# nghiapq77/face-recognition-cpp-tensorrt

Measured on AMD Instinct MI355X. Metric: faces/sec end-to-end (detect+embed+match), 640x640 batch=32, 1M gallery, higher is better.
Workload: dtype f16 MFMA recogniser convs (fp32 accumulate) + fp32-accurate detector (fp32 MFMA, fp16 hi/lo-split MFMA for the 64-channel 3x3 convs) + int8-screened coarse scan (fp16 MFMA on exactly widened int8 rows) + exact f32 re-rank match (bit-identical to the exact f32 scan)

## Files before the change

### face-recognition-cpp-tensorrt_amd/csrc/frt_kernels.h

```cpp
#pragma once
#include <hip/hip_runtime.h>
#include <stdint.h>

#include <vector>

#include "../../include/frt.h"
#include "frt_faces.hpp"

typedef _Float16 half_t;
typedef _Float16 half8 __attribute__((ext_vector_type(8)));
typedef _Float16 half4 __attribute__((ext_vector_type(4)));
typedef float floatx16 __attribute__((ext_vector_type(16)));
typedef float floatx4 __attribute__((ext_vector_type(4)));

constexpr int FRT_MAX_DEVICES = 32;
inline bool frt_first_use_on_device(bool (&done)[FRT_MAX_DEVICES]) {
    int d = 0;
    (void)hipGetDevice(&d);
    d &= FRT_MAX_DEVICES - 1;
    if (done[d]) return false;
    done[d] = true;
    return true;
}

void launch_spin(double microseconds, hipStream_t s);
double launch_mfma_probe(int mix, int n_wg, int iters, const void *src, float *out, hipStream_t s);

struct MatchPartial {
    float sim;
    int32_t idx;
};
template <typename GT>
void launch_match_top1(const GT *rows, int N, int D, const float *queries, int F, MatchPartial *partial, int partial_blocks, int32_t *idx_out,
                       float *sim_out, int row_offset, hipStream_t s);
int match_top1_blocks(int N, int F);
template <typename GT>
void launch_match_full(const GT *rows, int N, int D, const float *queries, int F, float *out, hipStream_t s);
constexpr int FRT_MATCH_COARSE_WG = 256;
constexpr int FRT_MATCH_SEL_SUB = 64;
constexpr int FRT_MATCH_CTL_WORDS = 32 + FRT_MATCH_SEL_SUB * 32;
struct MatchPair {
    int q, tile;
};
constexpr int FRT_MATCH_PAIR_TILE_MASK = (1 << 28) - 1;
constexpr int FRT_MATCH_CTL_OVERFLOW = 1, FRT_MATCH_CTL_SEG0 = 32, FRT_MATCH_CTL_STRIDE = 32;
struct ScreenScratch {
    float *tilemax;
    float *wgmax;
    void *pairs;
    int pair_cap;
    int *ctl;
    unsigned long long *qkey;
    const uint8_t *g8;
    const float *g8_scale;
    float gerr;
};
size_t gallery8_bytes(int N, int D);
void launch_gallery_shadow8(const float *gallery, int N, int D, uint8_t *g8, float *scale, int *max_err2_bits, int *max_norm2_bits, hipStream_t s);
void launch_gallery_shadow(const float *gallery, int N, int D, half_t *g16, int *max_norm2_bits, hipStream_t s);
void launch_match_screened(const float *gallery, const half_t *g16, int N, int D, const float *queries, int F, int k, float gmax_norm,
                           const ScreenScratch &w, float *kth_scratch, MatchPartial *partial, int partial_blocks, int32_t *idx_out, float *sim_out,
                           int row_offset, hipStream_t s);
void launch_match_topk(const float *gallery, const half_t *g16, int N, int D, const float *queries, int F, int k, bool screen, float gmax_norm,
                       const ScreenScratch &w, float *kth_scratch, MatchPartial *partial, int partial_blocks, int32_t *idx_out, float *sim_out,
                       int row_offset, hipStream_t s);
int match_topk_max();
bool launch_match_coarse(const half_t *g16, int N, int D, const float *queries, int F, const ScreenScratch &w, hipStream_t s);
void launch_match_select_threshold(int N, int D, const float *queries, int F, float threshold, int tile_min, float gmax_norm, const ScreenScratch &w, bool i8,
                                   hipStream_t s);
void launch_match_topk_labels(const float *gallery, const half_t *g16, int N, int D, const float *queries, int F, int k, int kth_count, float gmax_norm,
                              const ScreenScratch &w, float *kth_scratch, MatchPartial *partial, int partial_blocks, const int32_t *labels,
                              int32_t *label_out, int32_t *idx_out, float *sim_out, int row_offset, hipStream_t s);
void launch_half_to_float(const half_t *in, long n, float *out, hipStream_t s);
void launch_float_to_half(const float *in, long n, half_t *out, hipStream_t s);
void launch_merge_topk(const int32_t *idx_all, const float *sim_all, int shards, int n, int k, int32_t *idx_out, float *sim_out, hipStream_t s);
void launch_merge_topk_labels(const int32_t *label_all, const int32_t *idx_all, const float *sim_all, int shards, int n, int k, int32_t *label_out,
                              int32_t *idx_out, float *sim_out, hipStream_t s);
size_t gallery16_elems(int N, int D);
__device__ __forceinline__ long g16_index(long g, int k, int D) {
    return ((((g >> 7) * 4 + ((g >> 5) & 3)) * (long)(D >> 4) + (k >> 4)) * 64 + ((k >> 3) & 1) * 32 + (g & 31)) * 8 + (k & 7);
}
__device__ __forceinline__ floatx4 load_g4(const float *G, long g, int D, int k) { return *reinterpret_cast<const floatx4 *>(G + g * D + k); }
__device__ __forceinline__ floatx4 load_g4(const half_t *G, long g, int D, int k) {
    const half4 h = *reinterpret_cast<const half4 *>(G + g16_index(g, k, D));
    return floatx4{(float)h[0], (float)h[1], (float)h[2], (float)h[3]};
}
template <typename GT>
__device__ __forceinline__ float exact_row_dot(const GT *__restrict__ G, long g, int D, const float *q) {
    float acc = 0.f;
#pragma unroll 8
    for (int k0 = 0; k0 < D; k0 += 8) {
        const floatx4 a = load_g4(G, g, D, k0), b = load_g4(G, g, D, k0 + 4);
        const floatx4 x = *reinterpret_cast<const floatx4 *>(q + k0), y = *reinterpret_cast<const floatx4 *>(q + k0 + 4);
#pragma unroll
        for (int s2 = 0; s2 < 4; ++s2) {
            acc = __builtin_fmaf(a[s2], x[s2], acc);
            acc = __builtin_fmaf(b[s2], y[s2], acc);
        }
    }
    return acc;
}
bool match_screen_supported(int D);
void launch_rows_to_half(const float *in, long row0, long n_rows, int D, half_t *g16, hipStream_t s);
template <typename GT>
void launch_rows_norm(const GT *G, int row0, int n_rows, int D, int *max_norm2_bits, hipStream_t s);
void launch_gallery_shadow8_rows(const float *rows, int row0, int n_rows, uint8_t *g8, float *scale, int *max_err2_bits, int *max_norm2_bits, hipStream_t s);
void launch_gather_rows(const float *G, int D, int a, int n_rows, const int *keys, int klo, int khi, float *bounce, hipStream_t s);
void launch_gather_rows16(const half_t *G, int D, long tile0, long n_tiles, int n_new, const int *keys, int klo, int khi, half_t *bounce, hipStream_t s);

void launch_cluster_init(int32_t *parent, int N, long long *stats, hipStream_t s);
void launch_cluster_queries(const half_t *rows, int row0, int n, int D, float *out, hipStream_t s);
template <typename GT>
void launch_cluster_rerank_union(const GT *rows, int N, int D, const float *queries, int q_row0, int tile_origin, const ScreenScratch &w, float t,
                                 int32_t *parent, long long *stats, int *chunk_overflow, hipStream_t s);
void launch_cluster_dense_union(const float *full, int F, int N, int q_row0, float t, int32_t *parent, long long *stats, hipStream_t s);
void launch_cluster_flatten(const int32_t *parent, int N, int32_t *labels, long long *stats, long long screened_chunks, long long dense_chunks,
                            hipStream_t s);

constexpr int FRT_SEPARATION_MAX_THRESHOLDS = 64;
void launch_match_select_kth(int N, int D, const float *queries, int F, int kth_count, float gmax_norm, const ScreenScratch &w, float *kth_scratch, bool i8,
                             hipStream_t s);
void launch_match_top1_excluding(const float *gallery, const half_t *g16, int N, int D, const float *queries, int F, bool screened, const ScreenScratch &w,
                                 MatchPartial *partial, int partial_blocks, const int32_t *labels, const int32_t *excluded, int32_t *idx_out, float *sim_out,
                                 int *overflow_out, hipStream_t s);
template <typename GT>
void launch_separation_genuine(const GT *rows, int N, int D, const int *group_off, const int *group_rows, const int *pos_ident, float *gen_sim,
                               int32_t *gen_row, hipStream_t s);
void launch_separation_reduce(const float *gen_sim, const int32_t *gen_row, const float *imp_sim, const int32_t *imp_row, int N, const float *thresholds,
                              int n_thresholds, const int *chunk_overflow, int chunks, bool screened, long long *counts, long long *stats, hipStream_t s);

template <typename GT>
void launch_template_build(const GT *rows, int D, const int *group_off, const int *group_rows, int I, int row_offset, float *templates, float *min_sim,
                           int32_t *min_row, hipStream_t s);

constexpr int DET_MAX_LEVELS = 4, DET_MAX_SIZES = 3;
struct DetGeom {
    int in_w, in_h, frame_w, frame_h;
    int levels;
    int fw[DET_MAX_LEVELS], fh[DET_MAX_LEVELS];
    int base[DET_MAX_LEVELS];
    int nsz[DET_MAX_LEVELS];
    int min_size[DET_MAX_LEVELS][DET_MAX_SIZES];
    float step[DET_MAX_LEVELS];
    int A;
    float scale_w, scale_h;
    float nms_thr, bbox_thr;
    int max_faces;
};
DetGeom det_geometry(int family, int levels, int in_w, int in_h, int frame_w, int frame_h, float nms_threshold, float bbox_threshold, int max_faces);
struct Candidate {
    frt_bbox box;
    int32_t anchor;
};
void launch_decode(const float *loc, const float *conf, int n_frames, const DetGeom &g, Candidate *cand, int *cand_count, hipStream_t s);
void launch_nms(Candidate *cand, const float *loc, int *cand_count, int n_frames, const DetGeom &g, uint8_t *dead, frt_bbox *out, int *n_out,
                int *kept_anchor, hipStream_t s);
void launch_landmark_decode(const float *ldm, const int *kept_anchor, const int *n_out, int n_frames, const DetGeom &g, float *out, hipStream_t s);
void launch_align_faces(const uint8_t *frames, int frame_h, int frame_w, size_t row_stride, size_t frame_stride, const float *landmarks,
                        const int *n_boxes, int max_faces, int F, int frames_shared, uint8_t *crops, float *chw, int *valid, hipStream_t s);

void launch_det_preprocess(const uint8_t *frames, int n, int frame_h, int frame_w, size_t row_stride, size_t frame_stride, int in_h,
                           int in_w, float *out, hipStream_t s);
void launch_crop_faces(const uint8_t *frames, int frame_h, int frame_w, size_t row_stride, size_t frame_stride, const frt_bbox *boxes,
                       const int *n_boxes, int max_faces, int F, int frames_shared, int oh, int ow, uint8_t *crops, float *chw, int *valid,
                       hipStream_t s);
void launch_resize_linear(const uint8_t *src, int n, int sh, int sw, size_t sstride, size_t sframe, uint8_t *dst, int dh, int dw, size_t dstride,
                          size_t dframe, hipStream_t s);
void launch_face_normalize(const uint8_t *crops, int F, int oh, int ow, float *chw, hipStream_t s);
void launch_faces_prepare(const uint8_t *arena, const frt_face_desc *desc, int F, uint8_t *crops, float *chw, hipStream_t s);
void launch_images_resize(const uint8_t *arena, const frt_face_desc *desc, int n, int dh, int dw, uint8_t *out, hipStream_t s);

void launch_cut_tiles(const uint8_t *photo, int rows, int cols, size_t row_stride, const frt_tile *tiles, int n_tiles, int tile_rows, int tile_cols,
                      uint8_t *out, hipStream_t s);
struct TileMergeArgs {
    const frt_bbox *boxes;
    const int32_t *n_boxes;
    const frt_tile *tiles;
    int n_tiles, slots, photo_rows, photo_cols, tile_rows, tile_cols, metric, drop_cut;
    float thr;
    int max_out;
    unsigned long long *keys;
    frt_bbox *mbox;
    int *order;
    unsigned long long *mask;
    frt_bbox *out;
    int32_t *src_out;
    int *n_out;
};
size_t tile_merge_mask_words(int candidates);
void launch_tile_merge(const TileMergeArgs &a, hipStream_t s);
void launch_tile_landmarks(const float *ldm, const frt_tile *tiles, const int32_t *src, const int *n_out, int slots, int max_out, int photo_rows,
                           int photo_cols, int tile_rows, int tile_cols, float *out, hipStream_t s);
void launch_tile_faces_select(const frt_bbox *boxes, const int32_t *src, const float *ldm, const int *n_in, int cap, int min_face, int max_batch,
                              frt_bbox *boxes_kept, int32_t *src_kept, float *ldm_kept, int32_t *keep_pos, int *n_kept, int32_t *pass_count,
                              hipStream_t s);

void launch_enrol_select(const frt_face_result *results, const float *embeds, int n_frames, int max_faces, int32_t *status, frt_face_result *face_out,
                         float *rows, int32_t *count, hipStream_t s, const struct frt_face_quality *quality = nullptr);

void launch_face_quality(const uint8_t *crops, const frt_face_result *results, int n, const frt_quality_options &opt, struct frt_face_quality *out,
                         hipStream_t s);

struct DwPwArgs {
    const float *in; float *out;
    const float *wd, *bd;
    const float *wp, *bp;
    const float *add;
    int add_h, add_w;
    int B, Cin, H, W, Cout, Ho, Wo, stride, relu;
    float *tmp;
    const float *wd12;
    const half_t *wph;
    const float *wdp;
    const half_t *wpf;
    const float *wdt;
    const float *stem;
    const float *zeros;
};
size_t dwpw_wave_zero_bytes();
bool launch_dwpw_wave(const DwPwArgs &a, hipStream_t s);
void launch_dwpw(const DwPwArgs &a, hipStream_t s);
bool launch_dwpw_mfma(const DwPwArgs &a, hipStream_t s);
struct Conv3Args {
    const float *in; float *out;
    const float *w, *b;
    int B, Cin, H, W, Cout, Ho, Wo, stride, relu;
    int out_ctotal, out_coff;
    const half_t *wh;
    float *out2;
    int split, out2_ctotal, out2_coff;
};
void launch_conv3x3(const Conv3Args &a, hipStream_t s);
size_t det_stem_weight_floats();
void det_stem_pack(const Conv3Args &c, const DwPwArgs &d1, const DwPwArgs &d2, float *dst, hipStream_t s);
bool launch_det_stem(const uint8_t *frames, size_t row_stride, size_t frame_stride, const Conv3Args &c, const DwPwArgs &d1, const DwPwArgs &d2, hipStream_t s);
bool launch_det_conv1_u8(const uint8_t *frames, size_t row_stride, size_t frame_stride, const Conv3Args &a, hipStream_t s);
bool launch_conv3x3_split(const Conv3Args *a, int n, hipStream_t s);
void launch_conv3x3_multi(const Conv3Args *a, int n, hipStream_t s);
struct HeadArgs {
    const float *in;
    const float *wb, *bb;
    const float *wc, *bc;
    float *loc, *conf;
    int B, C, H, W, A, base;
    const float *wl, *bl;
    float *ldm;
};
void launch_heads(const HeadArgs &a, hipStream_t s);
void launch_heads_multi(const HeadArgs *a, int n, hipStream_t s);

struct SlimHeadArgs {
    const float *in;
    const float *wd;
    const float *wp, *bp;
    int C, H, W, na, base;
};
struct SlimHeadsArgs {
    SlimHeadArgs lv[3];
    float *loc, *conf, *ldm;
    int B, A;
};
void launch_slim_heads(const SlimHeadsArgs &a, int n, hipStream_t s);
struct DenseHeadArgs {
    const float *in;
    const float *w, *b;
    float *loc, *conf, *ldm;
    int B, C, H, W, na, cout, cpad, A, base;
};
void launch_dense_head(const DenseHeadArgs &a, hipStream_t s);
struct RfbProjArgs {
    const float *in;
    const float *w, *b;
    float *red, *sc;
    int B, H, W;
};
void launch_rfb_proj(const RfbProjArgs &a, hipStream_t s);
struct RfbConvArgs {
    const float *in; float *out;
    const float *w, *b;
    int Cin, Cout, dil, relu, in_ctotal, in_coff, out_ctotal, out_coff;
};
struct RfbConvMulti {
    RfbConvArgs p[3];
    int B, H, W;
};
void launch_rfb_conv(const RfbConvMulti &a, int n, hipStream_t s);
struct RfbTailArgs {
    const float *cat;
    const float *w, *b;
    const float *sc;
    float *out;
    float scale;
    int B, H, W;
};
void launch_rfb_tail(const RfbTailArgs &a, hipStream_t s);

enum { EPI_PRELU = 0, EPI_BN = 1, EPI_BN_ADD_BN = 2, EPI_PARTIAL = 3, EPI_BN_SE = 4 };
struct ConvMfmaArgs {
    const half_t *x;
    const half_t *w;
    const half_t *wf;
    const half_t *wf2;
    int B, H, W, Cin, Ho, Wo, Cout, ks, stride, pad;
    int mode;
    const float *p0, *p1, *p2, *p3;
    const half_t *sc;
    int sc_h, sc_w, sc_stride;
    const half_t *scx;
    const half_t *wscf;
    const float *psc0, *psc1;
    int Csc;
    half_t *out0, *out1;
    float *outf;
    int splits;
    const half_t *zeros;
    float *se_pool;
    const float *se_w1, *se_w2;
    int *se_counter;
    int se_flag_off;
    int se_epoch;
    int *se_error;
    const int *strip_tab;
    int strip_period, strip_ppx;
};
struct StripGeometry {
    int H, W;
    int compact;
    int linear;
    int nt;
    int R;
    int n_img;
    int nslot;
    int threads;
};
struct StripTables {
    int period = 0;
    int ppx = 0;
    int stride = 0;
    std::vector<int> data;
};
constexpr int strip_table_stride(const StripGeometry &g) { return g.nslot * g.threads + g.nt * 64 + (g.compact ? g.nt * 4 : g.nt * 32); }
StripTables strip_tables(const StripGeometry &g);
enum ConvFamily { CONV_SMALL, CONV_KS, CONV_C64, CONV_S2, CONV_STRIP };
struct ConvPlan {
    int family = CONV_STRIP;
    int row = 0;
    const char *label = "";
    int R = 0, n_img = 1;
    int M = 0;
    bool uses_scx = false;
    int se_row = -1;
    const char *se_label = nullptr;
    bool se_fused() const { return se_row >= 0; }
    void take_se_tail() { row = se_row; label = se_label; }
};
struct ConvRow {
    const char *label;
    void (*launch)(const ConvMfmaArgs &a, const ConvPlan &p, hipStream_t s);
    int se_row;
};
inline void conv_plan_row(ConvPlan &p, int family, const ConvRow *table, int row) {
    p.family = family;
    p.row = row;
    p.label = table[row].label;
}
inline void conv_plan_se_twin(ConvPlan &p, const ConvRow *table, const ConvMfmaArgs &a) {
    if (table[p.row].se_row < 0 || a.mode != EPI_BN_ADD_BN || !a.se_pool || !a.sc || !a.out1) return;
    p.se_row = table[p.row].se_row;
    p.se_label = table[p.se_row].label;
}
ConvPlan conv_plan(const ConvMfmaArgs &a);
bool conv_strip_geometry(const ConvMfmaArgs &a, const ConvPlan &p, StripGeometry &g);
void conv_strip_tables_warm(const ConvMfmaArgs &a, const ConvPlan &p);
void launch_conv_mfma(const ConvMfmaArgs &a, const ConvPlan &p, hipStream_t s);
bool conv_se_fits_device();
bool plan_small(const ConvMfmaArgs &a, ConvPlan &p);
void launch_small(const ConvMfmaArgs &a, const ConvPlan &p, hipStream_t s);
bool plan_ks(const ConvMfmaArgs &a, ConvPlan &p);
void launch_ks(const ConvMfmaArgs &a, const ConvPlan &p, hipStream_t s);
bool plan_c64(const ConvMfmaArgs &a, ConvPlan &p);
void launch_c64(const ConvMfmaArgs &a, const ConvPlan &p, hipStream_t s);
bool plan_s2(const ConvMfmaArgs &a, ConvPlan &p);
void launch_s2(const ConvMfmaArgs &a, const ConvPlan &p, hipStream_t s);
struct ArcInputArgs {
    const float *x;
    const float *w;
    const float *s0, *b0;
    const float *slope;
    const float *s1, *b1;
    half_t *y, *z;
    int F, H, W;
    const half_t *wh;
};
void launch_arc_input(const ArcInputArgs &a, hipStream_t s);
bool launch_arc_input_mfma(const ArcInputArgs &a, hipStream_t s);
void launch_fc_slices(const half_t *z, const half_t *wfrag, int F, float *partial, hipStream_t s);
struct Conv32Args {
    const float *x, *w, *ps, *pb;
    float *out;
    int F, H, W, Cin, Ho, Wo, Cout, ks, stride, pad, mode;
    const float *p0, *p1, *sc;
    int sc_h, sc_w, sc_stride;
};
void launch_arc32_input(const float *x, const float *w, const float *s0, const float *b0, const float *slope, float *y, int F, hipStream_t s);
void launch_conv32(const Conv32Args &c, hipStream_t s);
void pack_conv32_weights(const float *w, int cout, int taps, int cin, float *out);
void launch_fc32(const float *y, const float *sn, const float *bn, const float *w, float *out, int F, hipStream_t s);
void launch_se32(const float *res, const float *w1, const float *w2, float *gate, const float *sc, float *out, int F, int Ho, int Wo, int C, int sc_h, int sc_w, int sc_stride,
                 hipStream_t s);
void launch_fc_finalize(const float *partial, int splits, int F, const float *bias, const float *s, const float *b, const int *valid,
                        float *out, hipStream_t s_);
void launch_arc_flip_pair(const float *chw, float *pair, int n, hipStream_t s);
void launch_arc_flip_mirror(const float *chw, float *mirror, int n, hipStream_t s);
void launch_fc_finalize_pair(const float *partial_a, const float *partial_b, int splits, int rows, int n, const float *bias, const float *s, const float *b,
                             const int *valid, float *out, hipStream_t s_);
struct SeArgs {
    const half_t *res;
    const float *w1;
    const float *w2;
    const half_t *sc; int sc_h, sc_w, sc_stride;
    const float *s1, *b1;
    half_t *y, *z;
    float *pool;
    float *gate;
    int F, H, W, C;
    int *counter;
};
void launch_se(const SeArgs &a, hipStream_t s);

constexpr int FRT_TRACK_MAX_FRAMES = 256, FRT_TRACK_MAX_STREAMS = 1024, FRT_TRACK_MAX_SLOTS = 64, FRT_TRACK_MAX_DIM = 2048;
struct TrackStreamIds {
    uint16_t id[FRT_TRACK_MAX_FRAMES];
};
struct TrackArgs {
    frt_track_state *slots;
    float *sums;
    int32_t *counters;
    int max_tracks, max_faces, dim;
    float iou_threshold, decay;
    int max_missed, min_hits;
    const frt_face_result *results;
    const float *embeds;
    frt_track_result *tracks;
    float *templates;
    float reid_threshold, iou_min_sim;
    float *sim;
    unsigned long long *sim_defined;
    frt_track_assoc *assoc;
};
void launch_track_similarity(const TrackArgs &a, const TrackStreamIds &ids, int n_frames, hipStream_t s);
void launch_track_update(const TrackArgs &a, const TrackStreamIds &ids, int n_frames, bool appearance, hipStream_t s);
void launch_track_identity(const TrackArgs &a, const TrackStreamIds &ids, int n_frames, const int32_t *idx, const float *sim, hipStream_t s);
void launch_track_reset(const TrackArgs &a, int n_streams, int stream, hipStream_t s);
```

### face-recognition-cpp-tensorrt_amd/csrc/kernels_det_wave.hip

```cpp
#include <cstdlib>
#include <type_traits>
#include <utility>

#include "frt_kernels.h"

namespace {

typedef float floatx2 __attribute__((ext_vector_type(2)));
typedef _Float16 half2v __attribute__((ext_vector_type(2)));
typedef unsigned uint2v __attribute__((ext_vector_type(2)));
typedef unsigned uint4v __attribute__((ext_vector_type(4)));
typedef unsigned uint16v __attribute__((ext_vector_type(16)));

__device__ __forceinline__ int xcd_tile(int nblocks) {
    const int bq = nblocks >> 3, brem = nblocks & 7;
    const int xcd = blockIdx.x & 7, slot = blockIdx.x >> 3;
    return (xcd < brem ? xcd * (bq + 1) : brem * (bq + 1) + (xcd - brem) * bq) + slot;
}

template <int CIN, int NCB, int H, int W, int STRIDE, int NBUF_>
struct WaveGeom {
    static constexpr int WO = W / STRIDE, HO = H / STRIDE;
    static constexpr int HW = H * W, HOWO = HO * WO;
    static constexpr int SPAN = (WO + 62) / WO + 1;
    static constexpr int ROWS = STRIDE * (SPAN - 1) + 3;
    static constexpr int SL = W / 4 + 1;
    static constexpr int CPC = 8;
    static constexpr int SPC = CPC / 4;
    static constexpr int CHS = SL * 16;
    static constexpr int ROWB = CPC * CHS + (W % 32) * 4;
    static constexpr int CHUNKB = ROWS * ROWB;
    static constexpr int NDR = (CPC * SL + 63) / 64;
    static constexpr int DMAOPS = ROWS * NDR;
    static constexpr int NBUF = NBUF_, LA = NBUF_ - 1;
    static constexpr int NCHUNK = CIN / CPC, NG = CIN / 16, NSTEP = CIN / 4;
    static constexpr int NA = 2 * NCB;
    static constexpr int LDS_BYTES = NBUF * CHUNKB + 16;
    static_assert(SPC == 2 && CIN % 16 == 0 && CHS / 4 + 2 < 256 && LA >= 2, "shape not covered");
    static constexpr int younger(int cw) {
        const int at_step = cw == 0 ? -1 : 2 * cw - 2;
        int n = 0;
        bool seen = false;
        for (int k = 0; k < LA; ++k) {
            if (seen) n += DMAOPS;
            if (k == cw) seen = true;
        }
        if (seen) n += NA;
        for (int st = 0; st <= at_step; ++st) {
            if ((st & 1) == 0 && st / 2 + LA < NCHUNK) {
                if (seen) n += DMAOPS;
                if (st / 2 + LA == cw) seen = true;
            }
            if (st < at_step && (st & 3) == 3 && st / 4 + 1 < NG && seen) n += NA;
        }
        return n;
    }
};

template <int I, int N, class F>
__device__ __forceinline__ void static_for(F &&f) {
    if constexpr (I < N) {
        f(std::integral_constant<int, I>{});
        static_for<I + 1, N>(f);
    }
}

template <int N>
__device__ __forceinline__ void wait_vm() {
    static_assert(N >= 0 && N < 64, "vmcnt is a 6-bit counter");
#ifdef WAVE_VM0
    asm volatile("s_waitcnt vmcnt(0)" ::: "memory");
#else
    asm volatile("s_waitcnt vmcnt(%0)" ::"n"(N) : "memory");
#endif

}

struct WaveArgs {
    const float *in; float *out;
    const float *bp, *wdp;
    const half_t *wpf;
    const float *zeros;
#ifdef WAVE_STAMP
    long long *stamps;
#endif
};
#ifdef WAVE_STAMP
#define WSTAMP(i) do { if (blockIdx.x == 0 && threadIdx.x == 0) a.stamps[i] = __builtin_readcyclecounter(); } while (0)
#else
#define WSTAMP(i) do { } while (0)
#endif

template <int CIN, int COUT, int NCB, int H, int W, int STRIDE, int NBUF>
__global__ __launch_bounds__(64) __attribute__((amdgpu_num_sgpr(48))) void dwpw_wave_kernel(WaveArgs a) {
    using G = WaveGeom<CIN, NCB, H, W, STRIDE, NBUF>;
    extern __shared__ __attribute__((aligned(16))) char lds[];
    const int lane = threadIdx.x, r = lane & 31, hi = lane >> 5;
    constexpr int HW = G::HW, HoWo = G::HOWO;
    constexpr int tpi = (HoWo + 63) >> 6;
    const int lid = xcd_tile(gridDim.x);
    const int b = lid / tpi, p0 = (lid - b * tpi) * 64;
    const int y_first = p0 / G::WO;
    const int cob = (int)blockIdx.y * NCB;

    WSTAMP(0);
    for (int o = lane * 16; o < G::LDS_BYTES; o += 1024) *reinterpret_cast<floatx4 *>(lds + o) = floatx4{0.f, 0.f, 0.f, 0.f};
    asm volatile("s_waitcnt lgkmcnt(0)" ::: "memory");

    unsigned voff[G::NDR];
    bool lval[G::NDR];
#pragma unroll
    for (int i = 0; i < G::NDR; ++i) {
        const int q = lane + 64 * i, k = q / G::SL, sl = q - k * G::SL;
        lval[i] = q < G::CPC * G::SL && sl >= 1;
        voff[i] = lval[i] ? (unsigned)((k * HW + (sl - 1) * 4) * 4) : 0u;
    }
    const char *rsrc[G::ROWS];
    unsigned rstep[G::ROWS];
    {
        const char *inb = reinterpret_cast<const char *>(a.in + (long)b * CIN * HW);
        const char *zer = reinterpret_cast<const char *>(a.zeros);
#pragma unroll
        for (int j = 0; j < G::ROWS; ++j) {
            const int iy = y_first * STRIDE - 1 + j;
            const bool in = iy >= 0 && iy < H;
            rsrc[j] = in ? inb + iy * W * 4 : zer;
            rstep[j] = in ? (unsigned)(G::CPC * HW * 4) : 0u;
        }
    }
    const unsigned lds0 = (unsigned)(uintptr_t)(__attribute__((address_space(3))) char *)lds;
    auto dma_chunk = [&](auto cc) {
        constexpr int c = decltype(cc)::value;
#pragma unroll
        for (int i = 0; i < G::NDR; ++i)
            if (lval[i]) {
                const unsigned vo = voff[i];
#pragma unroll
                for (int j = 0; j < G::ROWS; ++j) {
                    const char *src = rsrc[j];
                    const unsigned dst = lds0 + (c % G::NBUF) * G::CHUNKB + j * G::ROWB + i * 1024;
                    asm volatile("s_mov_b32 m0, %2\n\tglobal_load_lds_dwordx4 %0, %1" ::"v"(vo), "s"(src), "s"(dst) : "memory");
                }
            }
#pragma unroll
        for (int j = 0; j < G::ROWS; ++j) rsrc[j] += rstep[j];
    };

    const int pl = min(p0 + lane, HoWo - 1);
    const int oy = pl / G::WO, ox = pl - oy * G::WO;
    const unsigned rb = (unsigned)(uintptr_t)(__attribute__((address_space(3))) char *)lds +
                        (unsigned)(((oy - y_first) * STRIDE) * G::ROWB + (ox * STRIDE + 3) * 4);

    half8 ah[2][NCB], al[2][NCB];
    const half_t *wf = a.wpf + (long)lane * 8;
    const int ncb_total = COUT / 32;
    auto load_a = [&](auto gc) {
        constexpr int g = decltype(gc)::value;
#pragma unroll
        for (int cb = 0; cb < NCB; ++cb) {
            const half_t *p = wf + ((long)(g * ncb_total + cob + cb) * 2) * 512;
            ah[g & 1][cb] = *reinterpret_cast<const half8 *>(p);
            al[g & 1][cb] = *reinterpret_cast<const half8 *>(p + 512);
        }
    };

    floatx16 acc[2][NCB];
#pragma unroll
    for (int t = 0; t < 2; ++t)
#pragma unroll
        for (int cb = 0; cb < NCB; ++cb)
#pragma unroll
            for (int e = 0; e < 16; ++e) acc[t][cb][e] = 0.f;

    floatx4 bias4[NCB][4];
    WSTAMP(1);
    asm volatile("" ::: "memory");
    static_for<0, G::LA>(dma_chunk);
    asm volatile("" ::: "memory");
    load_a(std::integral_constant<int, 0>{});
    asm volatile("" ::: "memory");

    floatx2 tv[2][2][9];
    auto issue_taps3 = [&](auto qc, auto dc, floatx2(&v)[9]) {
        constexpr int q = decltype(qc)::value, d = decltype(dc)::value;
        constexpr int c = q / (G::CPC / 2), pr = q % (G::CPC / 2);
        constexpr int boff = (c % G::NBUF) * G::CHUNKB + 2 * pr * G::CHS + d * G::ROWB;
        const unsigned b0 = rb + boff;
        asm volatile("ds_read2_b32 %0, %3 offset0:0 offset1:%4\n"
                     "ds_read2_b32 %1, %3 offset0:1 offset1:%5\n"
                     "ds_read2_b32 %2, %3 offset0:2 offset1:%6"
                     : "=&v"(v[3 * d]), "=&v"(v[3 * d + 1]), "=&v"(v[3 * d + 2])
                     : "v"(b0), "n"(G::CHS / 4), "n"(G::CHS / 4 + 1), "n"(G::CHS / 4 + 2)
                     : "memory");
    };
    auto issue_taps = [&](auto qc, floatx2(&v)[9]) {
        issue_taps3(qc, std::integral_constant<int, 0>{}, v);
        issue_taps3(qc, std::integral_constant<int, 1>{}, v);
        issue_taps3(qc, std::integral_constant<int, 2>{}, v);
    };
    auto landed = [&](floatx2(&u)[9], floatx2(&v)[9]) {
        asm volatile("s_waitcnt lgkmcnt(0)"
                     : "+v"(u[0]), "+v"(u[1]), "+v"(u[2]), "+v"(u[3]), "+v"(u[4]), "+v"(u[5]), "+v"(u[6]), "+v"(u[7]), "+v"(u[8])::"memory");
        asm volatile("" : "+v"(v[0]), "+v"(v[1]), "+v"(v[2]), "+v"(v[3]), "+v"(v[4]), "+v"(v[5]), "+v"(v[6]), "+v"(v[7]), "+v"(v[8])::"memory");
    };
#define WAVE_W_CLOBBERS                                                                                                                            \
    "s56", "s57", "s58", "s59", "s60", "s61", "s62", "s63", "s64", "s65", "s66", "s67", "s68", "s69", "s70", "s71", "s72", "s73", "s74", "s75", "s76", \
        "s77", "s78", "s79", "s80", "s81", "s82", "s83", "s84", "s85", "s86", "s87", "s88", "s89", "s90", "s91", "s92", "s93", "s94", "s95"
    const float *wdp = a.wdp;
    auto load_w = [&](auto sc) {
        constexpr int st = decltype(sc)::value;
        const float *wsrc = wdp;
        asm volatile("s_load_dwordx16 s[56:71], %0, %1\n"
                     "s_load_dwordx4 s[72:75], %0, %2\n"
                     "s_load_dwordx16 s[76:91], %0, %3\n"
                     "s_load_dwordx4 s[92:95], %0, %4" ::"s"(wsrc),
                     "n"(st * 160), "n"(st * 160 + 64), "n"(st * 160 + 80), "n"(st * 160 + 144)
                     : "memory", WAVE_W_CLOBBERS);
    };
    const floatx2 ones = {1.f, 1.f};
    auto chain3 = [&](auto jc, floatx2 &oa, floatx2 &ob, floatx2(&u)[9], floatx2(&v)[9]) {
        constexpr int j = decltype(jc)::value;
        const floatx2 one2 = ones;
        if constexpr (j == 0)
            asm volatile("v_pk_mul_f32 %0, %8, s[74:75]\n"
                         "v_pk_mul_f32 %1, %8, s[94:95]\n"
                         "v_pk_fma_f32 %0, %2, s[56:57], %0\n"
                         "v_pk_fma_f32 %1, %5, s[76:77], %1\n"
                         "v_pk_fma_f32 %0, %3, s[58:59], %0\n"
                         "v_pk_fma_f32 %1, %6, s[78:79], %1\n"
                         "v_pk_fma_f32 %0, %4, s[60:61], %0\n"
                         "v_pk_fma_f32 %1, %7, s[80:81], %1"
                         : "=&v"(oa), "=&v"(ob)
                         : "v"(u[0]), "v"(u[1]), "v"(u[2]), "v"(v[0]), "v"(v[1]), "v"(v[2]), "v"(one2)
                         : "memory");
        else if constexpr (j == 1)
            asm volatile("v_pk_fma_f32 %0, %2, s[62:63], %0\n"
                         "v_pk_fma_f32 %1, %5, s[82:83], %1\n"
                         "v_pk_fma_f32 %0, %3, s[64:65], %0\n"
                         "v_pk_fma_f32 %1, %6, s[84:85], %1\n"
                         "v_pk_fma_f32 %0, %4, s[66:67], %0\n"
                         "v_pk_fma_f32 %1, %7, s[86:87], %1"
                         : "+v"(oa), "+v"(ob)
                         : "v"(u[3]), "v"(u[4]), "v"(u[5]), "v"(v[3]), "v"(v[4]), "v"(v[5])
                         : "memory");
        else
            asm volatile("v_pk_fma_f32 %0, %2, s[68:69], %0\n"
                         "v_pk_fma_f32 %1, %5, s[88:89], %1\n"
                         "v_pk_fma_f32 %0, %3, s[70:71], %0\n"
                         "v_pk_fma_f32 %1, %6, s[90:91], %1\n"
                         "v_pk_fma_f32 %0, %4, s[72:73], %0\n"
                         "v_pk_fma_f32 %1, %7, s[92:93], %1"
                         : "+v"(oa), "+v"(ob)
                         : "v"(u[6]), "v"(u[7]), "v"(u[8]), "v"(v[6]), "v"(v[7]), "v"(v[8])
                         : "memory");
    };

    {
        const float *wsrc = wdp;
        static_for<0, (CIN * 10 * 4 + 63) / 64>([&](auto ic) {
            unsigned sink;
            const float *src2 = wsrc;
            asm volatile("s_load_dword %0, %1, %2" : "=s"(sink) : "s"(src2), "n"(decltype(ic)::value * 64) : "memory");
        });
        asm volatile("s_waitcnt lgkmcnt(0)" ::: "memory");
    }
    WSTAMP(2);
    wait_vm<G::younger(0)>();
    asm volatile("s_sleep 2" ::: "memory");
    WSTAMP(3);
    load_w(std::integral_constant<int, 0>{});
    issue_taps(std::integral_constant<int, 0>{}, tv[0][0]);
    issue_taps(std::integral_constant<int, 1>{}, tv[0][1]);

    unsigned hp[8], lp[8];
    half8 pbh[2], pbl[2];
    constexpr int MF_STEP = 3 * 2 * NCB / 4;
    auto mfma_n = [&](auto gc, auto mc) {
        constexpr int g = decltype(gc)::value, m = decltype(mc)::value;
        constexpr int round = m / (2 * NCB), t = (m / NCB) % 2, cb = m % NCB;
#ifndef WAVE_NO_MFMA
        acc[t][cb] = __builtin_amdgcn_mfma_f32_32x32x16_f16(round == 2 ? al[g & 1][cb] : ah[g & 1][cb], round == 1 ? pbl[t] : pbh[t], acc[t][cb], 0, 0, 0);
#else
        acc[t][cb][round] += (float)pbh[t][cb] + (float)pbl[t][cb] + (float)ah[g & 1][cb][round] + (float)al[g & 1][cb][round];
#endif
    };
    auto step = [&](auto sc) {
        constexpr int st = decltype(sc)::value;
        constexpr int c = st / 2, g = st / 4, k = st % 4;
        if constexpr ((st & 1) == 0 && c + G::LA < G::NCHUNK) dma_chunk(std::integral_constant<int, c + G::LA>{});
        if constexpr ((st & 1) == 0 && c + 1 < G::NCHUNK) wait_vm<G::younger(c + 1)>();
        if constexpr (st == G::NSTEP - 2) {
#pragma unroll
            for (int cb = 0; cb < NCB; ++cb)
#pragma unroll
                for (int kq = 0; kq < 4; ++kq) bias4[cb][kq] = *reinterpret_cast<const floatx4 *>(a.bp + (cob + cb) * 32 + 8 * kq + 4 * hi);
        }
        WSTAMP(7 + st);
        floatx2 oa, ob;
        landed(tv[st & 1][0], tv[st & 1][1]);
        chain3(std::integral_constant<int, 0>{}, oa, ob, tv[st & 1][0], tv[st & 1][1]);
        chain3(std::integral_constant<int, 1>{}, oa, ob, tv[st & 1][0], tv[st & 1][1]);
        chain3(std::integral_constant<int, 2>{}, oa, ob, tv[st & 1][0], tv[st & 1][1]);
        if constexpr (st + 1 < G::NSTEP) load_w(std::integral_constant<int, st + 1>{});
        static_for<0, 6>([&](auto ic) {
            constexpr int i = decltype(ic)::value;
            if constexpr (g > 0)
                static_for<i * MF_STEP / 6, (i + 1) * MF_STEP / 6>(
                    [&](auto mc) { mfma_n(std::integral_constant<int, g - 1>{}, std::integral_constant<int, k * MF_STEP + decltype(mc)::value>{}); });
            if constexpr (st + 1 < G::NSTEP) issue_taps3(std::integral_constant<int, 2 * st + 2 + i / 3>{}, std::integral_constant<int, i % 3>{}, tv[(st + 1) & 1][i / 3]);
            __builtin_amdgcn_sched_barrier(0);
        });
#pragma unroll
        for (int pr = 0; pr < 2; ++pr) {
            floatx2 o = pr ? ob : oa;
            asm("v_max_f32 %0, 0, %0" : "+v"(o[0]));
            asm("v_max_f32 %0, 0, %0" : "+v"(o[1]));
            const half2v h = __builtin_convertvector(o, half2v);
            float l0 = (float)h[0], l1 = (float)h[1];
            asm("v_sub_f32 %0, %1, %0" : "+v"(l0) : "v"(o[0]));
            asm("v_sub_f32 %0, %1, %0" : "+v"(l1) : "v"(o[1]));
            const half2v l = __builtin_convertvector(floatx2{l0, l1}, half2v);
            hp[2 * k + pr] = __builtin_bit_cast(unsigned, h);
            lp[2 * k + pr] = __builtin_bit_cast(unsigned, l);
        }
        if constexpr (k == 3) {
#pragma unroll
            for (int i = 0; i < 4; ++i) {
                const uint2v sh = __builtin_amdgcn_permlane32_swap(hp[i], hp[4 + i], false, false);
                const uint2v sl = __builtin_amdgcn_permlane32_swap(lp[i], lp[4 + i], false, false);
                hp[i] = sh[0];
                hp[4 + i] = sh[1];
                lp[i] = sl[0];
                lp[4 + i] = sl[1];
            }
#pragma unroll
            for (int t = 0; t < 2; ++t) {
                pbh[t] = __builtin_bit_cast(half8, uint4v{hp[4 * t], hp[4 * t + 1], hp[4 * t + 2], hp[4 * t + 3]});
                pbl[t] = __builtin_bit_cast(half8, uint4v{lp[4 * t], lp[4 * t + 1], lp[4 * t + 2], lp[4 * t + 3]});
            }
            asm volatile("" ::: "memory");
            if constexpr (g + 1 < G::NG) load_a(std::integral_constant<int, g + 1>{});
            asm volatile("" ::: "memory");
        }
        __builtin_amdgcn_sched_barrier(0);
    };
    static_for<0, G::NSTEP>(step);
    static_for<0, 4 * MF_STEP>([&](auto mc) { mfma_n(std::integral_constant<int, G::NG - 1>{}, mc); });
    WSTAMP(4);

#pragma unroll
    for (int t = 0; t < 2; ++t) {
        const int pix = p0 + 32 * t + r;
        if (pix >= HoWo) continue;
        float *ob = a.out + ((long)b * COUT + cob * 32 + 4 * hi) * HoWo + pix;
#pragma unroll
        for (int cb = 0; cb < NCB; ++cb)
#pragma unroll
            for (int e = 0; e < 16; ++e) {
                float v = acc[t][cb][e] + bias4[cb][e >> 2][e & 3];
                asm("v_max_f32 %0, 0, %0" : "+v"(v));
                ob[(long)(cb * 32 + (e & 3) + 8 * (e >> 2)) * HoWo] = v;
            }
    }
    WSTAMP(5);
}

template <int CIN, int COUT, int NCB, int H, int W, int STRIDE, int NBUF>
void launch_wave(const DwPwArgs &a, hipStream_t s) {
    using G = WaveGeom<CIN, NCB, H, W, STRIDE, NBUF>;
    static bool once = [] {
        (void)hipFuncSetAttribute(reinterpret_cast<const void *>(&dwpw_wave_kernel<CIN, COUT, NCB, H, W, STRIDE, NBUF>), hipFuncAttributeMaxDynamicSharedMemorySize,
                                  G::LDS_BYTES);
        return true;
    }();
    (void)once;
    constexpr int tpi = (G::HOWO + 63) / 64;
#ifdef WAVE_STAMP
    const WaveArgs w{a.in, a.out, a.bp, a.wdp, a.wpf, a.zeros, reinterpret_cast<long long *>(a.tmp)};
#else
    const WaveArgs w{a.in, a.out, a.bp, a.wdp, a.wpf, a.zeros};
#endif
    hipLaunchKernelGGL((dwpw_wave_kernel<CIN, COUT, NCB, H, W, STRIDE, NBUF>), dim3((unsigned)(a.B * tpi), COUT / (32 * NCB)), dim3(64), G::LDS_BYTES, s, w);
}


}

size_t dwpw_wave_zero_bytes() { return (size_t)1 << 20; }

bool launch_dwpw_wave(const DwPwArgs &a, hipStream_t s) {
    if (!a.wdp || !a.wpf || !a.zeros || a.add || !a.wd || !a.relu) return false;
    if (a.W != a.Wo * a.stride || (a.stride == 1 ? a.H != a.Ho : a.H != 2 * a.Ho)) return false;
    if ((long)a.B * a.Cin * a.H * a.W * 4 >= (1L << 31)) return false;
    if (a.stride == 1 && a.Cin == 128 && a.Cout == 128 && a.W == 40 && a.H == 40 && a.B >= 12) {
        launch_wave<128, 128, 4, 40, 40, 1, 3>(a, s);
        return true;
    }
    if (a.stride == 1 && a.Cin == 64 && a.Cout == 64 && a.W == 80 && a.H == 80 && a.B >= 3) {
        launch_wave<64, 64, 2, 80, 80, 1, 3>(a, s);
        return true;
    }
    if (a.stride == 1 && a.Cin == 256 && a.Cout == 256 && a.W == 20 && a.H == 20 && a.B >= 12) {
        launch_wave<256, 256, 2, 20, 20, 1, 4>(a, s);
        return true;
    }
    return false;
}
```

Before: 44880.

## Split depthwise input channels across waves and share pointwise fragments via LDS

For the 256-channel 20x20 detector layer, the fused depthwise+pointwise wave kernel now runs four waves per workgroup. Each wave computes the depthwise output for a quarter of the input channels, writes the hi/lo fp16 fragments to LDS, and after a barrier each wave runs the full-K pointwise MFMA for its own cout blocks. Previously every cout-block group recomputed the whole depthwise conv separately. The 64-channel 80x80 layer also switches to 4-channel DMA chunks, which shrinks its LDS footprint for higher occupancy. The risks are a workgroup barrier, larger LDS use per block, and a serialized pointwise phase after the depthwise phase.

```diff
diff --git a/face-recognition-cpp-tensorrt_amd/csrc/frt_kernels.h b/face-recognition-cpp-tensorrt_amd/csrc/frt_kernels.h
--- a/face-recognition-cpp-tensorrt_amd/csrc/frt_kernels.h
+++ b/face-recognition-cpp-tensorrt_amd/csrc/frt_kernels.h
@@ -219,6 +219,14 @@
 };
 size_t dwpw_wave_zero_bytes();
 bool launch_dwpw_wave(const DwPwArgs &a, hipStream_t s);
+struct DwPwWavePlan {
+    const char *kernel;
+    int waves;
+    int lds_bytes;
+    int wg_per_cu;
+    int waves_per_simd;
+};
+int dwpw_wave_plans(DwPwWavePlan *out, int cap);
 void launch_dwpw(const DwPwArgs &a, hipStream_t s);
 bool launch_dwpw_mfma(const DwPwArgs &a, hipStream_t s);
 struct Conv3Args {
diff --git a/face-recognition-cpp-tensorrt_amd/csrc/kernels_det_wave.hip b/face-recognition-cpp-tensorrt_amd/csrc/kernels_det_wave.hip
--- a/face-recognition-cpp-tensorrt_amd/csrc/kernels_det_wave.hip
+++ b/face-recognition-cpp-tensorrt_amd/csrc/kernels_det_wave.hip
@@ -18,14 +18,16 @@
     return (xcd < brem ? xcd * (bq + 1) : brem * (bq + 1) + (xcd - brem) * bq) + slot;
 }
 
-template <int CIN, int NCB, int H, int W, int STRIDE, int NBUF_>
+template <int CIN, int NCB, int H, int W, int STRIDE, int NBUF_, int NW_ = 1, int CPC_ = 8>
 struct WaveGeom {
+    static constexpr int NW = NW_;
+    static constexpr int CINW = CIN / NW_;
     static constexpr int WO = W / STRIDE, HO = H / STRIDE;
     static constexpr int HW = H * W, HOWO = HO * WO;
     static constexpr int SPAN = (WO + 62) / WO + 1;
     static constexpr int ROWS = STRIDE * (SPAN - 1) + 3;
     static constexpr int SL = W / 4 + 1;
-    static constexpr int CPC = 8;
+    static constexpr int CPC = CPC_;
     static constexpr int SPC = CPC / 4;
     static constexpr int CHS = SL * 16;
     static constexpr int ROWB = CPC * CHS + (W % 32) * 4;
@@ -33,12 +35,15 @@
     static constexpr int NDR = (CPC * SL + 63) / 64;
     static constexpr int DMAOPS = ROWS * NDR;
     static constexpr int NBUF = NBUF_, LA = NBUF_ - 1;
-    static constexpr int NCHUNK = CIN / CPC, NG = CIN / 16, NSTEP = CIN / 4;
-    static constexpr int NA = 2 * NCB;
-    static constexpr int LDS_BYTES = NBUF * CHUNKB + 16;
-    static_assert(SPC == 2 && CIN % 16 == 0 && CHS / 4 + 2 < 256 && LA >= 2, "shape not covered");
+    static constexpr int NCHUNK = CINW / CPC, NG = CINW / 16, NSTEP = CINW / 4;
+    static constexpr int NGT = CIN / 16;
+    static constexpr int NA = NW == 1 ? 2 * NCB : 0;
+    static constexpr int RING_BYTES = NBUF * CHUNKB + 16;
+    static constexpr int FRAG_BYTES = NW == 1 ? 0 : NGT * 4096;
+    static constexpr int LDS_BYTES = NW * RING_BYTES + FRAG_BYTES;
+    static_assert((SPC == 1 || SPC == 2) && CIN % (16 * NW) == 0 && CHS / 4 + 2 < 256 && LA >= 2 && RING_BYTES % 16 == 0 && NCHUNK >= LA, "shape not covered");
     static constexpr int younger(int cw) {
-        const int at_step = cw == 0 ? -1 : 2 * cw - 2;
+        const int at_step = cw == 0 ? -1 : SPC * cw - SPC;
         int n = 0;
         bool seen = false;
         for (int k = 0; k < LA; ++k) {
@@ -47,9 +52,9 @@
         }
         if (seen) n += NA;
         for (int st = 0; st <= at_step; ++st) {
-            if ((st & 1) == 0 && st / 2 + LA < NCHUNK) {
+            if (st % SPC == 0 && st / SPC + LA < NCHUNK) {
                 if (seen) n += DMAOPS;
-                if (st / 2 + LA == cw) seen = true;
+                if (st / SPC + LA == cw) seen = true;
             }
             if (st < at_step && (st & 3) == 3 && st / 4 + 1 < NG && seen) n += NA;
         }
@@ -91,20 +96,23 @@
 #define WSTAMP(i) do { } while (0)
 #endif
 
-template <int CIN, int COUT, int NCB, int H, int W, int STRIDE, int NBUF>
-__global__ __launch_bounds__(64) __attribute__((amdgpu_num_sgpr(48))) void dwpw_wave_kernel(WaveArgs a) {
-    using G = WaveGeom<CIN, NCB, H, W, STRIDE, NBUF>;
-    extern __shared__ __attribute__((aligned(16))) char lds[];
-    const int lane = threadIdx.x, r = lane & 31, hi = lane >> 5;
+template <int CIN, int COUT, int NCB, int H, int W, int STRIDE, int NBUF, int NW, int CPC>
+__global__ __launch_bounds__(64 * NW) __attribute__((amdgpu_num_sgpr(48))) void dwpw_wave_kernel(WaveArgs a) {
+    using G = WaveGeom<CIN, NCB, H, W, STRIDE, NBUF, NW, CPC>;
+    static_assert(NW == 1 || COUT == 32 * NCB * NW, "NW > 1: the waves of a tile share out all 32-cout blocks");
+    extern __shared__ __attribute__((aligned(16))) char lds_all[];
+    const int lane = threadIdx.x & 63, r = lane & 31, hi = lane >> 5;
+    const int wv = NW == 1 ? 0 : __builtin_amdgcn_readfirstlane((int)threadIdx.x >> 6);
+    char *const lds = lds_all + wv * G::RING_BYTES;
     constexpr int HW = G::HW, HoWo = G::HOWO;
     constexpr int tpi = (HoWo + 63) >> 6;
     const int lid = xcd_tile(gridDim.x);
     const int b = lid / tpi, p0 = (lid - b * tpi) * 64;
     const int y_first = p0 / G::WO;
-    const int cob = (int)blockIdx.y * NCB;
+    const int cob = (NW == 1 ? (int)blockIdx.y : wv) * NCB;
 
     WSTAMP(0);
-    for (int o = lane * 16; o < G::LDS_BYTES; o += 1024) *reinterpret_cast<floatx4 *>(lds + o) = floatx4{0.f, 0.f, 0.f, 0.f};
+    for (int o = lane * 16; o < G::RING_BYTES; o += 1024) *reinterpret_cast<floatx4 *>(lds + o) = floatx4{0.f, 0.f, 0.f, 0.f};
     asm volatile("s_waitcnt lgkmcnt(0)" ::: "memory");
 
     unsigned voff[G::NDR];
@@ -118,7 +126,7 @@
     const char *rsrc[G::ROWS];
     unsigned rstep[G::ROWS];
     {
-        const char *inb = reinterpret_cast<const char *>(a.in + (long)b * CIN * HW);
+        const char *inb = reinterpret_cast<const char *>(a.in + ((long)b * CIN + wv * G::CINW) * HW);
         const char *zer = reinterpret_cast<const char *>(a.zeros);
 #pragma unroll
         for (int j = 0; j < G::ROWS; ++j) {
@@ -128,7 +136,7 @@
             rstep[j] = in ? (unsigned)(G::CPC * HW * 4) : 0u;
         }
     }
-    const unsigned lds0 = (unsigned)(uintptr_t)(__attribute__((address_space(3))) char *)lds;
+    const unsigned lds0 = (unsigned)(uintptr_t)(__attribute__((address_space(3))) char *)lds_all + (unsigned)(wv * G::RING_BYTES);
     auto dma_chunk = [&](auto cc) {
         constexpr int c = decltype(cc)::value;
 #pragma unroll
@@ -148,8 +156,7 @@
 
     const int pl = min(p0 + lane, HoWo - 1);
     const int oy = pl / G::WO, ox = pl - oy * G::WO;
-    const unsigned rb = (unsigned)(uintptr_t)(__attribute__((address_space(3))) char *)lds +
-                        (unsigned)(((oy - y_first) * STRIDE) * G::ROWB + (ox * STRIDE + 3) * 4);
+    const unsigned rb = lds0 + (unsigned)(((oy - y_first) * STRIDE) * G::ROWB + (ox * STRIDE + 3) * 4);
 
     half8 ah[2][NCB], al[2][NCB];
     const half_t *wf = a.wpf + (long)lane * 8;
@@ -177,7 +184,7 @@
     asm volatile("" ::: "memory");
     static_for<0, G::LA>(dma_chunk);
     asm volatile("" ::: "memory");
-    load_a(std::integral_constant<int, 0>{});
+    if constexpr (NW == 1) load_a(std::integral_constant<int, 0>{});
     asm volatile("" ::: "memory");
 
     floatx2 tv[2][2][9];
@@ -206,7 +213,7 @@
 #define WAVE_W_CLOBBERS                                                                                                                            \
     "s56", "s57", "s58", "s59", "s60", "s61", "s62", "s63", "s64", "s65", "s66", "s67", "s68", "s69", "s70", "s71", "s72", "s73", "s74", "s75", "s76", \
         "s77", "s78", "s79", "s80", "s81", "s82", "s83", "s84", "s85", "s86", "s87", "s88", "s89", "s90", "s91", "s92", "s93", "s94", "s95"
-    const float *wdp = a.wdp;
+    const float *wdp = a.wdp + wv * (G::CINW / 2) * 20;
     auto load_w = [&](auto sc) {
         constexpr int st = decltype(sc)::value;
         const float *wsrc = wdp;
@@ -257,7 +264,7 @@
 
     {
         const float *wsrc = wdp;
-        static_for<0, (CIN * 10 * 4 + 63) / 64>([&](auto ic) {
+        static_for<0, (G::CINW * 10 * 4 + 63) / 64>([&](auto ic) {
             unsigned sink;
             const float *src2 = wsrc;
             asm volatile("s_load_dword %0, %1, %2" : "=s"(sink) : "s"(src2), "n"(decltype(ic)::value * 64) : "memory");
@@ -274,6 +281,7 @@
 
     unsigned hp[8], lp[8];
     half8 pbh[2], pbl[2];
+    char *const frag = lds_all + NW * G::RING_BYTES + lane * 16;
     constexpr int MF_STEP = 3 * 2 * NCB / 4;
     auto mfma_n = [&](auto gc, auto mc) {
         constexpr int g = decltype(gc)::value, m = decltype(mc)::value;
@@ -286,10 +294,10 @@
     };
     auto step = [&](auto sc) {
         constexpr int st = decltype(sc)::value;
-        constexpr int c = st / 2, g = st / 4, k = st % 4;
-        if constexpr ((st & 1) == 0 && c + G::LA < G::NCHUNK) dma_chunk(std::integral_constant<int, c + G::LA>{});
-        if constexpr ((st & 1) == 0 && c + 1 < G::NCHUNK) wait_vm<G::younger(c + 1)>();
-        if constexpr (st == G::NSTEP - 2) {
+        constexpr int c = st / G::SPC, g = st / 4, k = st % 4;
+        if constexpr (st % G::SPC == 0 && c + G::LA < G::NCHUNK) dma_chunk(std::integral_constant<int, c + G::LA>{});
+        if constexpr (st % G::SPC == 0 && c + 1 < G::NCHUNK) wait_vm<G::younger(c + 1)>();
+        if constexpr (NW == 1 && st == G::NSTEP - 2) {
 #pragma unroll
             for (int cb = 0; cb < NCB; ++cb)
 #pragma unroll
@@ -304,7 +312,7 @@
         if constexpr (st + 1 < G::NSTEP) load_w(std::integral_constant<int, st + 1>{});
         static_for<0, 6>([&](auto ic) {
             constexpr int i = decltype(ic)::value;
-            if constexpr (g > 0)
+            if constexpr (NW == 1 && g > 0)
                 static_for<i * MF_STEP / 6, (i + 1) * MF_STEP / 6>(
                     [&](auto mc) { mfma_n(std::integral_constant<int, g - 1>{}, std::integral_constant<int, k * MF_STEP + decltype(mc)::value>{}); });
             if constexpr (st + 1 < G::NSTEP) issue_taps3(std::integral_constant<int, 2 * st + 2 + i / 3>{}, std::integral_constant<int, i % 3>{}, tv[(st + 1) & 1][i / 3]);
@@ -333,19 +341,74 @@
                 lp[i] = sl[0];
                 lp[4 + i] = sl[1];
             }
+            if constexpr (NW == 1) {
+#pragma unroll
+                for (int t = 0; t < 2; ++t) {
+                    pbh[t] = __builtin_bit_cast(half8, uint4v{hp[4 * t], hp[4 * t + 1], hp[4 * t + 2], hp[4 * t + 3]});
+                    pbl[t] = __builtin_bit_cast(half8, uint4v{lp[4 * t], lp[4 * t + 1], lp[4 * t + 2], lp[4 * t + 3]});
+                }
+                asm volatile("" ::: "memory");
+                if constexpr (g + 1 < G::NG) load_a(std::integral_constant<int, g + 1>{});
+                asm volatile("" ::: "memory");
+            } else {
+                uint4v *fd = reinterpret_cast<uint4v *>(frag + ((wv * G::NG + g) * 4) * 1024);
+#pragma unroll
+                for (int t = 0; t < 2; ++t) {
+                    fd[64 * t] = uint4v{hp[4 * t], hp[4 * t + 1], hp[4 * t + 2], hp[4 * t + 3]};
+                    fd[64 * (2 + t)] = uint4v{lp[4 * t], lp[4 * t + 1], lp[4 * t + 2], lp[4 * t + 3]};
+                }
+            }
+        }
+        __builtin_amdgcn_sched_barrier(0);
+    };
+    static_for<0, G::NSTEP>(step);
+    if constexpr (NW == 1) {
+        static_for<0, 4 * MF_STEP>([&](auto mc) { mfma_n(std::integral_constant<int, G::NG - 1>{}, mc); });
+    } else {
+#pragma unroll
+        for (int cb = 0; cb < NCB; ++cb)
+#pragma unroll
+            for (int kq = 0; kq < 4; ++kq) bias4[cb][kq] = *reinterpret_cast<const floatx4 *>(a.bp + (cob + cb) * 32 + 8 * kq + 4 * hi);
+        constexpr int AD = 3;
+        half8 cah[4][NCB], cal[4][NCB];
+        auto load_ca = [&](auto gc) {
+            constexpr int g = decltype(gc)::value;
+#pragma unroll
+            for (int cb = 0; cb < NCB; ++cb) {
+                const half_t *p = wf + ((long)(g * ncb_total + cob + cb) * 2) * 512;
+                cah[g & 3][cb] = *reinterpret_cast<const half8 *>(p);
+                cal[g & 3][cb] = *reinterpret_cast<const half8 *>(p + 512);
+            }
+        };
+        static_for<0, AD>(load_ca);
+        asm volatile("s_waitcnt lgkmcnt(0)" ::: "memory");
+        __builtin_amdgcn_s_barrier();
+        asm volatile("" ::: "memory");
+        WSTAMP(6);
+        half8 bh[2][2], bl[2][2];
+        auto load_b = [&](auto gc) {
+            constexpr int g = decltype(gc)::value;
+            const half8 *fs = reinterpret_cast<const half8 *>(frag + g * 4096);
 #pragma unroll
             for (int t = 0; t < 2; ++t) {
-                pbh[t] = __builtin_bit_cast(half8, uint4v{hp[4 * t], hp[4 * t + 1], hp[4 * t + 2], hp[4 * t + 3]});
-                pbl[t] = __builtin_bit_cast(half8, uint4v{lp[4 * t], lp[4 * t + 1], lp[4 * t + 2], lp[4 * t + 3]});
-            }
-            asm volatile("" ::: "memory");
-            if constexpr (g + 1 < G::NG) load_a(std::integral_constant<int, g + 1>{});
-            asm volatile("" ::: "memory");
-        }
-        __builtin_amdgcn_sched_barrier(0);
-    };
-    static_for<0, G::NSTEP>(step);
-    static_for<0, 4 * MF_STEP>([&](auto mc) { mfma_n(std::integral_constant<int, G::NG - 1>{}, mc); });
+                bh[g & 1][t] = fs[64 * t];
+                bl[g & 1][t] = fs[64 * (2 + t)];
+            }
+        };
+        load_b(std::integral_constant<int, 0>{});
+        static_for<0, G::NGT>([&](auto gc) {
+            constexpr int g = decltype(gc)::value;
+            if constexpr (g + AD < G::NGT) load_ca(std::integral_constant<int, g + AD>{});
+            if constexpr (g + 1 < G::NGT) load_b(std::integral_constant<int, g + 1>{});
+            __builtin_amdgcn_sched_barrier(0);
+            static_for<0, 4 * MF_STEP>([&](auto mc) {
+                constexpr int m = decltype(mc)::value;
+                constexpr int round = m / (2 * NCB), t = (m / NCB) % 2, cb = m % NCB;
+                acc[t][cb] = __builtin_amdgcn_mfma_f32_32x32x16_f16(round == 2 ? cal[g & 3][cb] : cah[g & 3][cb], round == 1 ? bl[g & 1][t] : bh[g & 1][t], acc[t][cb], 0, 0, 0);
+            });
+            __builtin_amdgcn_sched_barrier(0);
+        });
+    }
     WSTAMP(4);
 
 #pragma unroll
@@ -365,11 +428,12 @@
     WSTAMP(5);
 }
 
-template <int CIN, int COUT, int NCB, int H, int W, int STRIDE, int NBUF>
+template <int CIN, int COUT, int NCB, int H, int W, int STRIDE, int NBUF, int NW, int CPC = 8>
 void launch_wave(const DwPwArgs &a, hipStream_t s) {
-    using G = WaveGeom<CIN, NCB, H, W, STRIDE, NBUF>;
+    using G = WaveGeom<CIN, NCB, H, W, STRIDE, NBUF, NW, CPC>;
+    static_assert(G::LDS_BYTES <= 160 * 1024, "more LDS than a CU has");
     static bool once = [] {
-        (void)hipFuncSetAttribute(reinterpret_cast<const void *>(&dwpw_wave_kernel<CIN, COUT, NCB, H, W, STRIDE, NBUF>), hipFuncAttributeMaxDynamicSharedMemorySize,
+        (void)hipFuncSetAttribute(reinterpret_cast<const void *>(&dwpw_wave_kernel<CIN, COUT, NCB, H, W, STRIDE, NBUF, NW, CPC>), hipFuncAttributeMaxDynamicSharedMemorySize,
                                   G::LDS_BYTES);
         return true;
     }();
@@ -380,7 +444,8 @@
 #else
     const WaveArgs w{a.in, a.out, a.bp, a.wdp, a.wpf, a.zeros};
 #endif
-    hipLaunchKernelGGL((dwpw_wave_kernel<CIN, COUT, NCB, H, W, STRIDE, NBUF>), dim3((unsigned)(a.B * tpi), COUT / (32 * NCB)), dim3(64), G::LDS_BYTES, s, w);
+    hipLaunchKernelGGL((dwpw_wave_kernel<CIN, COUT, NCB, H, W, STRIDE, NBUF, NW, CPC>), dim3((unsigned)(a.B * tpi), NW == 1 ? COUT / (32 * NCB) : 1), dim3(64 * NW),
+                       G::LDS_BYTES, s, w);
 }
 
 
@@ -393,16 +458,27 @@
     if (a.W != a.Wo * a.stride || (a.stride == 1 ? a.H != a.Ho : a.H != 2 * a.Ho)) return false;
     if ((long)a.B * a.Cin * a.H * a.W * 4 >= (1L << 31)) return false;
     if (a.stride == 1 && a.Cin == 128 && a.Cout == 128 && a.W == 40 && a.H == 40 && a.B >= 12) {
-        launch_wave<128, 128, 4, 40, 40, 1, 3>(a, s);
+        launch_wave<128, 128, 4, 40, 40, 1, 3, 1>(a, s);
         return true;
     }
     if (a.stride == 1 && a.Cin == 64 && a.Cout == 64 && a.W == 80 && a.H == 80 && a.B >= 3) {
-        launch_wave<64, 64, 2, 80, 80, 1, 3>(a, s);
+        launch_wave<64, 64, 2, 80, 80, 1, 3, 1, 4>(a, s);
         return true;
     }
     if (a.stride == 1 && a.Cin == 256 && a.Cout == 256 && a.W == 20 && a.H == 20 && a.B >= 12) {
-        launch_wave<256, 256, 2, 20, 20, 1, 4>(a, s);
+        launch_wave<256, 256, 2, 20, 20, 1, 4, 4>(a, s);
         return true;
     }
     return false;
 }
+
+int dwpw_wave_plans(DwPwWavePlan *out, int cap) {
+    const DwPwWavePlan plans[] = {
+        {"dwpw_wave_kernel<128, 128, 4, 40, 40, 1, 3, 1, 8>", 1, WaveGeom<128, 4, 40, 40, 1, 3, 1, 8>::LDS_BYTES, 4, 1},
+        {"dwpw_wave_kernel<64, 64, 2, 80, 80, 1, 3, 1, 4>", 1, WaveGeom<64, 2, 80, 80, 1, 3, 1, 4>::LDS_BYTES, 8, 2},
+        {"dwpw_wave_kernel<256, 256, 2, 20, 20, 1, 4, 4, 8>", 4, WaveGeom<256, 2, 20, 20, 1, 4, 4, 8>::LDS_BYTES, 1, 1},
+    };
+    const int n = (int)(sizeof plans / sizeof plans[0]);
+    for (int i = 0; i < n && i < cap; ++i) out[i] = plans[i];
+    return n;
+}
```

Result: no change. 45120 (median of 6 runs) (+0.5%).
